# sanje2v/DualSuperResLearningForSemSeg

Measured on AMD Instinct MI355X. Metric: stage-3 train images/sec at 256x512->512x1024, higher is better.
Workload: dtype f32; 1 GPU; DSRL stage 3 (ResNet-101 OS16 + ASPP + SSSR/SISR decoders + FA loss), full train step, random-init weights, 256x512 input -> 512x1024 logits; global_batch=8, per_gpu_batch=8, parallelism=dp1, optimizer=SGD m0.9 wd5e-4 lr0.006

## Files before the change

### dualsuperreslearningforsemseg_amd/csrc/bn.hip

```cpp
#include "common.h"
#include <algorithm>
#include <initializer_list>
#include <atomic>
#include <mutex>
#include <stdlib.h>

struct SeedArg { unsigned long long value; const unsigned long long* dev; };

namespace dsrl {

constexpr int kMaxRowBlocks = 256;

static int row_blocks(int64_t P) { return (int)std::max<int64_t>(1, std::min<int64_t>(kMaxRowBlocks, ceil_div(P, 32))); }

__global__ __launch_bounds__(256) void bn_partial_kernel(const float* __restrict__ x, int ld, long long P, int C, long long rows_per_block,
                                                          float* __restrict__ part, int nbx) {
    __shared__ float sh[3][256];
    const ChanMap m = chan_map(C, blockIdx.y);
    const long long row0 = blockIdx.x * rows_per_block, row1 = min(P, row0 + rows_per_block);
    float n = 0.f, s1 = 0.f, s2 = 0.f, k0 = 0.f;
    if (m.c >= 0) {
        long long p = row0 + m.slot;
        if (p < row1) k0 = x[p * ld + m.c];
#pragma unroll 4
// ... 1465 lines not shown
                                  float* dresidual, int lddr, int64_t P, int C, const float* mean, const float* invstd, const float* gamma,
                                  float* dgamma, float* dbeta, int relu, float drop_p, int training, float* stats, int stats_parts, uint32_t* dx_amax,
                                  dsrl_stream_t stream, const BnRes2* res2);
extern "C" int dsrl_bn_bwd_from_stats_drop(const float* x, int ldx, const float* y, int ldy, const float* dy, int lddy, float* dx, int lddx,
                                           float* dresidual, int lddr, int64_t P, int C, const float* mean, const float* invstd, const float* gamma,
                                           float* dgamma, float* dbeta, int relu, float drop_p, int training, float* stats, int stats_parts, uint32_t* dx_amax,
                                           dsrl_stream_t stream) {
    return bn_bwd_from_stats_impl(x, ldx, y, ldy, dy, lddy, dx, lddx, dresidual, lddr, P, C, mean, invstd, gamma, dgamma, dbeta, relu, drop_p, training, stats, stats_parts,
                                  dx_amax, stream, nullptr);
}
extern "C" int dsrl_bn_bwd_from_stats_res(const float* x, int ldx, const float* y, int ldy, const float* dy, int lddy, float* dx, int lddx,
                                          float* dresidual, int lddr, int64_t P, int C, const float* mean, const float* invstd, const float* gamma,
                                          float* dgamma, float* dbeta, int relu, float drop_p, int training, float* stats, int stats_parts, uint32_t* dx_amax,
                                          const float* res_x, int res_ldx, const float* res_mean, const float* res_invstd, float* res_stats, int res_parts,
                                          dsrl_stream_t stream) {
    DSRL_REQUIRE(dresidual && res_x && res_mean && res_invstd && res_stats && res_ldx >= C && res_ldx % 4 == 0 && ((uintptr_t)res_x % 16) == 0, DSRL_E_BADARG,
                 "bn_bwd_from_stats_res: the residual branch's input / statistics / partials buffer are required (stride a multiple of 4, 16-byte aligned)");
    DSRL_REQUIRE(res_parts > 0 && res_parts == dsrl_bn_bwd_from_stats_res_parts(P, C, stats_parts), DSRL_E_BADARG,
                 "bn_bwd_from_stats_res: this launch writes %d row blocks of sums, the caller expects %d (dsrl_bn_bwd_from_stats_res_parts)",
                 dsrl_bn_bwd_from_stats_res_parts(P, C, stats_parts), res_parts);
    const BnRes2 r2{res_x, res_ldx, res_mean, res_invstd, res_stats, res_parts};
    return bn_bwd_from_stats_impl(x, ldx, y, ldy, dy, lddy, dx, lddx, dresidual, lddr, P, C, mean, invstd, gamma, dgamma, dbeta, relu, drop_p, training, stats, stats_parts,
                                  dx_amax, stream, &r2);
}
static int bn_bwd_from_stats_impl(const float* x, int ldx, const float* y, int ldy, const float* dy, int lddy, float* dx, int lddx,
                                  float* dresidual, int lddr, int64_t P, int C, const float* mean, const float* invstd, const float* gamma,
                                  float* dgamma, float* dbeta, int relu, float drop_p, int training, float* stats, int stats_parts, uint32_t* dx_amax,
                                  dsrl_stream_t stream, const BnRes2* res2) {
    DSRL_REQUIRE(drop_p >= 0.f && drop_p < 1.f && (drop_p == 0.f || relu), DSRL_E_BADARG, "bn_bwd_from_stats_drop: dropout p=%f needs the ReLU mask (y > 0)", drop_p);
    const float ks = drop_p > 0.f ? 1.f / (1.f - drop_p) : 1.f;
    DSRL_REQUIRE(x && dy && dx && mean && invstd && gamma && stats && P > 0 && P < (1ll << 31) && C > 0, DSRL_E_BADARG, "bn_bwd_from_stats: bad arguments");
// ... 100 lines not shown
```

### dualsuperreslearningforsemseg_amd/csrc/conv_common.h

```cpp
#pragma once
#include "common.h"

namespace dsrl {

using f32x16 = __attribute__((ext_vector_type(16))) float;
using bf16x8 = __attribute__((ext_vector_type(8))) __bf16;
using bf16x4 = __attribute__((ext_vector_type(4))) __bf16;
using f16x8 = __attribute__((ext_vector_type(8))) _Float16;
using f16x4 = __attribute__((ext_vector_type(4))) _Float16;

template <bool F16> struct Plane;
template <> struct Plane<false> {
    using v4 = bf16x4; using v8 = bf16x8;
    static __device__ __forceinline__ v4 cvt(const float* r) { return v4{(__bf16)r[0], (__bf16)r[1], (__bf16)r[2], (__bf16)r[3]}; }
    static __device__ __forceinline__ void residual(float* r, v4 t) {
#pragma unroll
        for (int e = 0; e < 4; ++e) r[e] -= (float)t[e];
    }
    static __device__ __forceinline__ f32x16 mfma(v8 a, v8 b, f32x16 c) { return __builtin_amdgcn_mfma_f32_32x32x16_bf16(a, b, c, 0, 0, 0); }
};
__device__ __forceinline__ float f16_resid_lo(unsigned t, float r) { float d; asm("v_fma_mix_f32 %0, %1, -1.0, %2 op_sel:[0,0,0] op_sel_hi:[1,0,0]" : "=v"(d) : "v"(t), "v"(r)); return d; }
__device__ __forceinline__ float f16_resid_hi(unsigned t, float r) { float d; asm("v_fma_mix_f32 %0, %1, -1.0, %2 op_sel:[1,0,0] op_sel_hi:[1,0,0]" : "=v"(d) : "v"(t), "v"(r)); return d; }
template <> struct Plane<true> {
    using v4 = f16x4; using v8 = f16x8;
// ... 27 lines not shown
    int R, S, Ho, Wo;
    int stride, pad, dil;
    int M;
    int cchunks;
    int splits;
    long long slab;
    unsigned x_bytes, w_bytes, y_bytes;
    int mtiles, ntiles, xcd_remap;
    int kg;
    int accumulate;
    float* stats;
    const float* bn_x; const float* bn_y; const float* bn_mean; const float* bn_invstd; float* bstats;
    int bn_ldx, bn_ldy, bn_relu;
    float bn_gscale;
    int bn_fast;
    int par, Hh, Wh, pbm;
    const unsigned* amax_a; const unsigned* amax_b;
    int w_split;
    unsigned mHW, sHW, mW, sW, mNT, sNT;
    unsigned a_lo, b_lo;
    int planes;
    float* coop_slab; unsigned* tickets;
};
constexpr int kCoopMaxTiles = (kAmaxShardStride - 1) * kAmaxShards;
__host__ __device__ inline int coop_ticket_word(int t) { return kAmaxShardStride * (t / (kAmaxShardStride - 1)) + 1 + t % (kAmaxShardStride - 1); }
__device__ __forceinline__ int dgrad_pix(const ConvArgs& a, int m) {
    const int t = m / a.pbm, p2 = a.par * a.par, c = t % p2, j = (t / p2) * a.pbm + (m - t * a.pbm);
    const int hw = a.Hh * a.Wh, n = j / hw, r = j - n * hw, hh = r / a.Wh, wh = r - hh * a.Wh;
    const int ph = c / a.par, pw = c - ph * a.par;
    return (n * a.Ho + hh * a.par + ph) * a.Wo + wh * a.par + pw;
// ... 54 lines not shown
```

### dualsuperreslearningforsemseg_amd/csrc/conv_igemm.hip

```cpp
#include "common.h"
#include "conv_common.h"
#include <algorithm>
#include <atomic>
#include <stdlib.h>
#include <string.h>
#include <mutex>
#include <vector>

namespace dsrl {

static std::atomic<int> g_conv_precision{-1};
constexpr int BK = 32;
constexpr int LDS_LD = 36;

template <int MR, int NR, int WGM, int WGN, bool DGRAD, int MINW = 2, bool = false>
__global__ __launch_bounds__(256, MINW) void conv_igemm_f32_kernel(const ConvArgs a) {
    constexpr int BM = 32 * MR * WGM, BN = 32 * NR * WGN;
    constexpr int A_IT = BM / 32, B_IT = BN / 32;
    extern __shared__ __attribute__((aligned(16))) float smem[];

    const int tid = threadIdx.x;
    const int lane = tid & 63;
    const int wave = __builtin_amdgcn_readfirstlane(tid >> 6);
    const int wm = wave / WGN, wn = wave % WGN;
// ... 1453 lines not shown
    if (int e = bind_stream_device(st)) return e;
    hipLaunchKernelGGL(weight_transpose_batched_kernel, dim3((unsigned)ceil_div(total_tiles, (int64_t)kWtTilesPerBlock)), dim3(256), 0, st, (const long long*)table, n,
                       (long long)total_tiles);
    return launch_status("weight_transpose_batched_kernel");
}

extern "C" int dsrl_conv2d_filters_amax_segment_floats(void) { return kAmaxSegFloats; }
extern "C" int dsrl_conv2d_filters_amax_batched(const int64_t* table, int64_t nseg, dsrl_stream_t stream) {
    DSRL_REQUIRE(table && nseg > 0 && nseg < (1ll << 31), DSRL_E_BADARG, "conv2d_filters_amax_batched: bad arguments");
    hipStream_t st = (hipStream_t)stream;
    if (int e = bind_stream_device(st)) return e;
    hipLaunchKernelGGL(weight_amax_batched_kernel, dim3((unsigned)nseg), dim3(256), 0, st, (const long long*)table);
    return launch_status("weight_amax_batched_kernel");
}

struct DgradBn { const float* x; const float* y; const float* mean; const float* invstd; float* stats; int ldx, ldy, relu; float gscale = 1.f; };
static bool bn_y_ok(const float* y, int ldy, int relu, int N, int H, int W, int C) {
    if (relu == 2) return y != nullptr && C % 32 == 0 && (long long)ldy >= (long long)N * H * W && ((uintptr_t)y % 4) == 0;
    return relu == 0 || (relu == 1 && y != nullptr && ldy >= C);
}
static int dgrad_impl(const float* dy, int lddy, const float* w, const float* wt_in, float* dx, int lddx,
                      int N, int H, int W, int C, int K, int R, int S, int stride, int pad, int dil,
                      void* ws, size_t ws_bytes, dsrl_stream_t stream, int accumulate, const DgradBn* bn = nullptr,
                      const unsigned* dy_amax = nullptr, const unsigned* w_amax = nullptr, const void* wt_split = nullptr,
                      const void* dy_planes = nullptr, const void* wt_planes = nullptr) {
    if (int e = check_conv(dy, w, dx, N, H, W, C, K, R, S, stride, pad, dil)) return e;
    const int Kp = pad4(K);
    DSRL_REQUIRE(lddy % 4 == 0 && ((uintptr_t)dy % 16) == 0, DSRL_E_UNSUPPORTED,
                 "conv2d_dgrad: lddy (%d) must be a multiple of 4 and dy 16-byte aligned", lddy);
    DSRL_REQUIRE(lddy >= Kp && lddx >= C, DSRL_E_BADARG, "conv2d_dgrad: ld smaller than (padded) channel count");
    hipStream_t st = (hipStream_t)stream;
// ... 50 lines not shown
                           (const float*)slabs, p.splits, a.slab, p.M, C, (const float*)nullptr, dx, lddx, accumulate);
        return launch_status("splitk_reduce_kernel");
    }
    if (p.splits > 1) {
        a.coop_slab = slabs; a.tickets = const_cast<unsigned*>(a.amax_a);
        a.y_bytes = (unsigned)span_bytes(p.M, lddx, C);
    }
    a.y = dx; a.ldy = lddx; a.bias = nullptr; a.accumulate = accumulate;
    if (stride > 1 && conv_planes(PASS_DGRAD) && H % stride == 0 && W % stride == 0 && (W / stride) % 32 == 0 && knob("DSRL_DGRAD_PARITY", 1)) {
        int bm, bn_; cfg_dims(p.cfg, bm, bn_);
        const long long Mc = (long long)N * (H / stride) * (W / stride);
        if (Mc % bm == 0) { a.par = stride; a.Hh = H / stride; a.Wh = W / stride; a.pbm = bm; }
    }
    if (bn) {
        a.bn_x = bn->x; a.bn_y = bn->y; a.bn_mean = bn->mean; a.bn_invstd = bn->invstd; a.bstats = bn->stats; a.bn_ldx = bn->ldx; a.bn_ldy = bn->ldy; a.bn_relu = bn->relu;
        a.bn_gscale = bn->gscale;
        const bool y4 = bn->relu != 1 || (bn->ldy % 4 == 0 && ((uintptr_t)bn->y % 16) == 0);
        a.bn_fast = a.par == 0 && C % 4 == 0 && bn->ldx % 4 == 0 && y4 && ((uintptr_t)bn->x % 16) == 0 &&
                    ((uintptr_t)bn->mean % 16) == 0 && ((uintptr_t)bn->invstd % 16) == 0 && ((uintptr_t)bn->stats % 16) == 0;
    }
    return launch_igemm<true>(a, p.cfg, st);
}

extern "C" int dsrl_conv2d_dgrad(const float* dy, int lddy, const float* w, const float* wt_in, float* dx, int lddx,
                                 int N, int H, int W, int C, int K, int R, int S, int stride, int pad, int dil,
                                 void* ws, size_t ws_bytes, dsrl_stream_t stream) {
    return dgrad_impl(dy, lddy, w, wt_in, dx, lddx, N, H, W, C, K, R, S, stride, pad, dil, ws, ws_bytes, stream, 0);
}
extern "C" int dsrl_conv2d_dgrad_stats_parts(int N, int H, int W, int C, int K, int R, int S, int stride, int pad, int dil) {
    const int Ho = out_size(H, R, stride, pad, dil), Wo = out_size(W, S, stride, pad, dil);
    if (Ho <= 0 || Wo <= 0) return 0;
    const int npl = conv_planes(PASS_DGRAD);
    return fwd_stats_parts(plan_dgrad(N, Ho, Wo, pad4(K), C, R, S, H, W, npl, stride), npl, true);
}
// ... 204 lines not shown
                 dsrl_conv2d_dgrad_stats_parts(N, H, W, C, K, R, S, stride, pad, dil), stats_parts);
    DgradBn bn{bn_x, bn_y, bn_mean, bn_invstd, bstats, bn_ldx, bn_ldy, bn_relu};
    return dgrad_impl(dy, lddy, w, wt_in, dx, lddx, N, H, W, C, K, R, S, stride, pad, dil, ws, ws_bytes, stream, accumulate ? 1 : 0, &bn, dy_amax, w_amax, wt_split);
}
extern "C" int dsrl_conv2d_fwd_planes(const float* x, int ldx, const uint32_t* x_amax, const void* x_planes, const float* w, const uint32_t* w_amax, const void* w_split,
                                      const void* w_planes, const float* bias, float* y, int ldy, int N, int H, int W, int C, int K, int R, int S, int stride, int pad, int dil,
                                      void* ws, size_t ws_bytes, float* stats, int stats_parts, dsrl_stream_t stream) {
    return fwd_impl(x, ldx, w, bias, y, ldy, N, H, W, C, K, R, S, stride, pad, dil, ws, ws_bytes, stream, stats, stats_parts, x_amax, w_amax, w_split, x_planes, w_planes);
}
extern "C" int dsrl_conv2d_dgrad_planes(const float* dy, int lddy, const uint32_t* dy_amax, const void* dy_planes, const float* w, const float* wt_in, const uint32_t* w_amax,
                                        const void* wt_split, const void* wt_planes, float* dx, int lddx,
                                        int N, int H, int W, int C, int K, int R, int S, int stride, int pad, int dil,
                                        void* ws, size_t ws_bytes, const float* bn_x, int bn_ldx, const float* bn_y, int bn_ldy,
                                        const float* bn_mean, const float* bn_invstd, int bn_relu, float* bstats, int stats_parts, int accumulate,
                                        dsrl_stream_t stream) {
    return dsrl_conv2d_dgrad_planes_drop(dy, lddy, dy_amax, dy_planes, w, wt_in, w_amax, wt_split, wt_planes, dx, lddx, N, H, W, C, K, R, S, stride, pad, dil, ws, ws_bytes,
                                         bn_x, bn_ldx, bn_y, bn_ldy, bn_mean, bn_invstd, bn_relu, 0.f, bstats, stats_parts, accumulate, stream);
}
extern "C" int dsrl_conv2d_dgrad_planes_drop(const float* dy, int lddy, const uint32_t* dy_amax, const void* dy_planes, const float* w, const float* wt_in, const uint32_t* w_amax,
                                             const void* wt_split, const void* wt_planes, float* dx, int lddx,
                                             int N, int H, int W, int C, int K, int R, int S, int stride, int pad, int dil,
                                             void* ws, size_t ws_bytes, const float* bn_x, int bn_ldx, const float* bn_y, int bn_ldy,
                                             const float* bn_mean, const float* bn_invstd, int bn_relu, float bn_drop_p, float* bstats, int stats_parts, int accumulate,
                                             dsrl_stream_t stream) {
    DSRL_REQUIRE(bn_drop_p >= 0.f && bn_drop_p < 1.f && (bn_drop_p == 0.f || bn_relu), DSRL_E_BADARG, "conv2d_dgrad_planes_drop: dropout p=%f needs the ReLU mask (y > 0)", bn_drop_p);
    if (bstats == nullptr)
        return dgrad_impl(dy, lddy, w, wt_in, dx, lddx, N, H, W, C, K, R, S, stride, pad, dil, ws, ws_bytes, stream, accumulate ? 1 : 0, nullptr, dy_amax, w_amax, wt_split,
                          dy_planes, wt_planes);
    DSRL_REQUIRE(bn_x && bn_mean && bn_invstd && bn_ldx >= C && bn_y_ok(bn_y, bn_ldy, bn_relu, N, H, W, C), DSRL_E_BADARG, "conv2d_dgrad_planes: bad BatchNorm arguments");
    DSRL_REQUIRE(dsrl_conv2d_dgrad_stats_parts(N, H, W, C, K, R, S, stride, pad, dil) == stats_parts && stats_parts > 0, DSRL_E_BADARG,
                 "conv2d_dgrad_planes: this launch writes %d row blocks of partials, the caller expects %d",
                 dsrl_conv2d_dgrad_stats_parts(N, H, W, C, K, R, S, stride, pad, dil), stats_parts);
    DgradBn bn{bn_x, bn_y, bn_mean, bn_invstd, bstats, bn_ldx, bn_ldy, bn_relu};
    bn.gscale = bn_drop_p > 0.f ? 1.f / (1.f - bn_drop_p) : 1.f;
    return dgrad_impl(dy, lddy, w, wt_in, dx, lddx, N, H, W, C, K, R, S, stride, pad, dil, ws, ws_bytes, stream, accumulate ? 1 : 0, &bn, dy_amax, w_amax, wt_split,
                      dy_planes, wt_planes);
}
extern "C" int dsrl_conv2d_wgrad_amax(const float* x, int ldx, const uint32_t* x_amax, const float* dy, int lddy, const uint32_t* dy_amax, float* dw,
                                      int N, int H, int W, int C, int K, int R, int S, int stride, int pad, int dil,
                                      void* ws, size_t ws_bytes, dsrl_stream_t stream) {
    return wgrad_impl(x, ldx, dy, lddy, dw, N, H, W, C, K, R, S, stride, pad, dil, ws, ws_bytes, stream, x_amax, dy_amax);
}


namespace dsrl {
constexpr unsigned kGroupMagic = 0x44535247u;
constexpr int kGroupMaxProblems = 512, kGroupMaxLaunches = kNumCfg + 2;
constexpr int kCfgW3 = kNumCfg;
struct GroupLaunch { int cfg, first, count, grid; double flops, bytes; };
// ... 332 lines not shown
```

### dualsuperreslearningforsemseg_amd/csrc/conv_planes.hip

```cpp
#include "common.h"
#include "conv_common.h"
#include "lds_dma.h"
#include <algorithm>

namespace dsrl {

template <int NPL> struct PlaneMfma;
template <> struct PlaneMfma<2> {
    template <int MR, int NR>
    static __device__ __forceinline__ void run(f32x16 (&acc)[MR][NR], const f16x8 (&fa)[MR][2], const f16x8 (&fb)[NR][2]) {
#pragma unroll
        for (int sum = 1; sum >= 0; --sum)
#pragma unroll
            for (int pa = 0; pa <= sum; ++pa)
#pragma unroll
                for (int i = 0; i < MR; ++i)
#pragma unroll
                    for (int j = 0; j < NR; ++j)
                        acc[i][j] = __builtin_amdgcn_mfma_f32_32x32x16_f16(fa[i][pa], fb[j][sum - pa], acc[i][j], 0, 0, 0);
    }
};
template <> struct PlaneMfma<1> {
    template <int MR, int NR>
    static __device__ __forceinline__ void run(f32x16 (&acc)[MR][NR], const f16x8 (&fa)[MR][1], const f16x8 (&fb)[NR][1]) {
// ... 276 lines not shown
        const float bv = (a.bias != nullptr && kok) ? a.bias[k] : 0.f;
#pragma unroll
        for (int i = 0; i < MR; ++i) {
            const int mb32 = m0 + (wm * MR + i) * 32, mb = mb32 + rq;
            if (a.accumulate && a.splits == 1) {
                float old[EPG];
#pragma unroll
                for (int e = 0; e < EPG; ++e) {
                    const int m = mb + (e & 3) + 8 * (e >> 2);
                    const unsigned off = (kok && m < a.M) ? ((unsigned)m * (unsigned)a.ldy + (unsigned)k) * 4u : kOOB;
                    old[e] = __uint_as_float(__builtin_amdgcn_raw_buffer_load_b32(yr, (int)off, 0, 0));
                }
#pragma unroll
                for (int e = 0; e < EPG; ++e) share_add(i, j, e, old[e]);
            }
#pragma unroll
            for (int e = 0; e < EPG; ++e) {
                const int m = mb + (e & 3) + 8 * (e >> 2);
                const unsigned off = (kok && m < a.M) ? ((unsigned)m * (unsigned)a.ldy + (unsigned)k) * 4u : kOOB;
                __builtin_amdgcn_raw_buffer_store_b32(__float_as_uint(share(i, j, e) + bv), yr, (int)off, 0, 0);
            }
        }
    }
    bool bstats_done = false;
    if constexpr (DGRAD && KG == 1) {
        if (a.bstats != nullptr && (a.splits == 1) && a.bn_fast) {
            constexpr int TR = 32 * MR, TC = 32 * NR, CQ = TC / 4, RSTEP = 64 / CQ, NIT = TR / RSTEP, NB = NIT < 8 ? NIT : 8;
            float* wt = reinterpret_cast<float*>(smem) + (size_t)wave * TR * TC;
            __syncthreads();
#pragma unroll
// ... 21 lines not shown
                    if (a.bn_relu == 2) yv[u] = bn_mask4(ok ? bn_mask_word(a, kk, m) >> (kk & 31) : 15u);
                    else yv[u] = (ok && a.bn_relu) ? *reinterpret_cast<const float4*>(a.bn_y + (long long)m * a.bn_ldy + kk) : make_float4(1.f, 1.f, 1.f, 1.f);
                }
#pragma unroll
                for (int u = 0; u < NB; ++u) {
                    const int row = r0_ + RSTEP * (b0 + u);
                    if (kok4 && mrow0 + row < a.M) {
                        const float4 gv = *reinterpret_cast<const float4*>(wt + row * TC + 4 * c4);
                        const float gs = a.bn_gscale;
                        const float g0 = (a.bn_relu && !(yv[u].x > 0.f)) ? 0.f : gv.x * gs, g1 = (a.bn_relu && !(yv[u].y > 0.f)) ? 0.f : gv.y * gs;
                        const float g2 = (a.bn_relu && !(yv[u].z > 0.f)) ? 0.f : gv.z * gs, g3 = (a.bn_relu && !(yv[u].w > 0.f)) ? 0.f : gv.w * gs;
                        sg[0] += g0; sgx[0] += g0 * ((xv[u].x - mu4.x) * is4.x);
                        sg[1] += g1; sgx[1] += g1 * ((xv[u].y - mu4.y) * is4.y);
                        sg[2] += g2; sgx[2] += g2 * ((xv[u].z - mu4.z) * is4.z);
                        sg[3] += g3; sgx[3] += g3 * ((xv[u].w - mu4.w) * is4.w);
                    }
                }
            }
#pragma unroll
            for (int sft = CQ; sft < 64; sft <<= 1)
#pragma unroll
                for (int q = 0; q < 4; ++q) { sg[q] += __shfl_xor(sg[q], sft); sgx[q] += __shfl_xor(sgx[q], sft); }
            if (lane < CQ && kok4) {
                const int nparts = a.mtiles * WGM, part = tile_m * WGM + wm;
                float* o = a.bstats + (long long)part * a.K + kk;
                *reinterpret_cast<float4*>(o) = make_float4(sg[0], sg[1], sg[2], sg[3]);
                *reinterpret_cast<float4*>(o + (long long)nparts * a.K) = make_float4(sgx[0], sgx[1], sgx[2], sgx[3]);
            }
            bstats_done = true;
        }
// ... 14 lines not shown
#pragma unroll
                for (int e = 0; e < EPG; ++e) {
                    const int m = mb32 + rq + (e & 3) + 8 * (e >> 2);
                    const bool ok = kok && m < a.M;
                    const long long px = m;
                    xv[e] = ok ? a.bn_x[px * a.bn_ldx + k] : 0.f;
                    if (a.bn_relu == 2) yv[e] = (!ok || ((bn_mask_word(a, k, px) >> (k & 31)) & 1u)) ? 1.f : 0.f;
                    else yv[e] = (ok && a.bn_relu) ? a.bn_y[px * a.bn_ldy + k] : 1.f;
                }
#pragma unroll
                for (int e = 0; e < EPG; ++e) {
                    const int m = mb32 + rq + (e & 3) + 8 * (e >> 2);
                    if (kok && m < a.M) {
                        const float g = (a.bn_relu && !(yv[e] > 0.f)) ? 0.f : share(i, j, e) * a.bn_gscale;
                        sg += g; sgx += g * ((xv[e] - mu) * is);
                    }
                }
            }
            sg += __shfl_xor(sg, 32); sgx += __shfl_xor(sgx, 32);
            if (KG == 1) {
                if (lane < 32 && kok) {
                    float* o = a.bstats + (long long)part * a.K + k;
                    o[0] = sg; o[(long long)nparts * a.K] = sgx;
                }
            } else if (lane < 32) {
                ex[(((grp * NW + wave) * NR + j) * 2 + 0) * 32 + lane] = sg;
                ex[(((grp * NW + wave) * NR + j) * 2 + 1) * 32 + lane] = sgx;
            }
        }
        if constexpr (KG > 1) {
// ... 282 lines not shown
```

### dualsuperreslearningforsemseg_amd/csrc/conv_split_kernel.h

```cpp
#pragma once
#include "common.h"
#include "conv_common.h"

namespace dsrl {

template <int MR, int NR, int WGM, int WGN, bool DGRAD, int NPL, int KG = 1, int ARITH = 0, bool STR1 = false, bool COOP = false>
__global__ __launch_bounds__(64 * WGM * WGN * KG, KG == 1 ? 2 : 1)
void conv_igemm_split_kernel(const ConvArgs a) {
    const int stride = STR1 ? 1 : a.stride, par = STR1 ? 0 : a.par;
    constexpr bool F16 = ARITH != 0, PREB = ARITH == 2;
    constexpr int NT = 64 * WGM * WGN, RP = NT / 4;
    static_assert(NT == 256 || (NT == 512 && KG == 1), "4 waves per K group, or one group of 8 waves");
    static_assert(!F16 || NPL <= 2, "f16x3 carries two fp16 terms per operand, f16x1 one");
    using PT = Plane<F16>;
    using pl4 = typename PT::v4; using pl8 = typename PT::v8;
    const unsigned am_a = F16 ? amax_fetch(a.amax_a) : 0u, am_b = F16 ? amax_fetch(a.amax_b) : 0u;
    int sh_a = 0, sh_b = 0;
    constexpr int BM = 32 * MR * WGM, BN = 32 * NR * WGN;
    constexpr int A_IT = (BM + RP - 1) / RP, B_IT = (BN + RP - 1) / RP;
    constexpr int NV = A_IT + B_IT;
    constexpr bool FS = F16;
    constexpr int ROWB = FS ? 64 : 32;
    constexpr int STAGE = (BM + BN) * NPL * ROWB;
    extern __shared__ __attribute__((aligned(16))) float smem[];
// ... 444 lines not shown
#pragma unroll
        for (int i = 0; i < MR; ++i) {
            const int mb32 = m0 + (wm * MR + i) * 32, mb = mb32 + rq;
            const int pix0 = (DGRAD && par) ? dgrad_pix(a, min(mb32, a.M - 1)) : mb32, pst = (DGRAD && par) ? par : 1;
            if (a.accumulate && single) {
                float old[EPG];
#pragma unroll
                for (int e = 0; e < EPG; ++e) {
                    const int m = mb + (e & 3) + 8 * (e >> 2);
                    const unsigned off = (kok && m < a.M) ? ((unsigned)(pix0 + (m - mb32) * pst) * (unsigned)a.ldy + (unsigned)k) * 4u : kOOB;
                    old[e] = __uint_as_float(__builtin_amdgcn_raw_buffer_load_b32(yr, (int)off, 0, 0));
                }
#pragma unroll
                for (int e = 0; e < EPG; ++e) share_add(i, j, e, old[e]);
            }
#pragma unroll
            for (int e = 0; e < EPG; ++e) {
                const int m = mb + (e & 3) + 8 * (e >> 2);
                const unsigned off = (kok && m < a.M) ? ((unsigned)(pix0 + (m - mb32) * pst) * (unsigned)a.ldy + (unsigned)k) * 4u : kOOB;
                __builtin_amdgcn_raw_buffer_store_b32(__float_as_uint(share(i, j, e) + bv), yr, (int)off, 0, 0);
            }
        }
    }
    bool bstats_done = false;
    if constexpr (DGRAD && KG == 1) {
        if (a.bstats != nullptr && single && a.bn_fast) {
            constexpr int TR = 32 * MR, TC = 32 * NR, CQ = TC / 4, RSTEP = 64 / CQ, NIT = TR / RSTEP, NB = NIT < 8 ? NIT : 8;
            float* wt = reinterpret_cast<float*>(smem) + (size_t)wave * TR * TC;
            __syncthreads();
#pragma unroll
// ... 21 lines not shown
                    if (a.bn_relu == 2) yv[u] = bn_mask4(ok ? bn_mask_word(a, kk, m) >> (kk & 31) : 15u);
                    else yv[u] = (ok && a.bn_relu) ? *reinterpret_cast<const float4*>(a.bn_y + (long long)m * a.bn_ldy + kk) : make_float4(1.f, 1.f, 1.f, 1.f);
                }
#pragma unroll
                for (int u = 0; u < NB; ++u) {
                    const int row = r0_ + RSTEP * (b0 + u);
                    if (kok4 && mrow0 + row < a.M) {
                        const float4 gv = *reinterpret_cast<const float4*>(wt + row * TC + 4 * c4);
                        const float gs = a.bn_gscale;
                        const float g0 = (a.bn_relu && !(yv[u].x > 0.f)) ? 0.f : gv.x * gs, g1 = (a.bn_relu && !(yv[u].y > 0.f)) ? 0.f : gv.y * gs;
                        const float g2 = (a.bn_relu && !(yv[u].z > 0.f)) ? 0.f : gv.z * gs, g3 = (a.bn_relu && !(yv[u].w > 0.f)) ? 0.f : gv.w * gs;
                        sg[0] += g0; sgx[0] += g0 * ((xv[u].x - mu4.x) * is4.x);
                        sg[1] += g1; sgx[1] += g1 * ((xv[u].y - mu4.y) * is4.y);
                        sg[2] += g2; sgx[2] += g2 * ((xv[u].z - mu4.z) * is4.z);
                        sg[3] += g3; sgx[3] += g3 * ((xv[u].w - mu4.w) * is4.w);
                    }
                }
            }
#pragma unroll
            for (int sft = CQ; sft < 64; sft <<= 1)
#pragma unroll
                for (int q = 0; q < 4; ++q) { sg[q] += __shfl_xor(sg[q], sft); sgx[q] += __shfl_xor(sgx[q], sft); }
            if (lane < CQ && kok4) {
                const int nparts = a.mtiles * WGM, part = tile_m * WGM + wm;
                float* o = a.bstats + (long long)part * a.K + kk;
                *reinterpret_cast<float4*>(o) = make_float4(sg[0], sg[1], sg[2], sg[3]);
                *reinterpret_cast<float4*>(o + (long long)nparts * a.K) = make_float4(sgx[0], sgx[1], sgx[2], sgx[3]);
            }
            bstats_done = true;
        }
// ... 15 lines not shown
#pragma unroll
                for (int e = 0; e < EPG; ++e) {
                    const int m = mb32 + rq + (e & 3) + 8 * (e >> 2);
                    const bool ok = kok && m < a.M;
                    const long long px = pix0 + (m - mb32) * pst;
                    xv[e] = ok ? a.bn_x[px * a.bn_ldx + k] : 0.f;
                    if (a.bn_relu == 2) yv[e] = (!ok || ((bn_mask_word(a, k, px) >> (k & 31)) & 1u)) ? 1.f : 0.f;
                    else yv[e] = (ok && a.bn_relu) ? a.bn_y[px * a.bn_ldy + k] : 1.f;
                }
#pragma unroll
                for (int e = 0; e < EPG; ++e) {
                    const int m = mb32 + rq + (e & 3) + 8 * (e >> 2);
                    if (kok && m < a.M) {
                        const float g = (a.bn_relu && !(yv[e] > 0.f)) ? 0.f : share(i, j, e) * a.bn_gscale;
                        sg += g; sgx += g * ((xv[e] - mu) * is);
                    }
                }
            }
            sg += __shfl_xor(sg, 32); sgx += __shfl_xor(sgx, 32);
            if (KG == 1) {
                if (lane < 32 && kok) {
                    float* o = a.bstats + (long long)part * a.K + k;
                    o[0] = sg; o[(long long)nparts * a.K] = sgx;
                }
            } else if (lane < 32) {
                ex[(((grp * 4 + wave) * NR + j) * 2 + 0) * 32 + lane] = sg;
                ex[(((grp * 4 + wave) * NR + j) * 2 + 1) * 32 + lane] = sgx;
            }
        }
        if constexpr (KG > 1) {
// ... 80 lines not shown
```

### dualsuperreslearningforsemseg_amd/functional.py

```python
import contextlib
import ctypes
import math
import os
import sys
import weakref

import numpy as np

import torch

from . import _lib
from ._lib import call, knob, query, DsrlHipError

CL = torch.channels_last


_raw_stream = getattr(torch._C, '_cuda_getCurrentRawStream', None)
_raw_device = getattr(torch._C, '_cuda_getDevice', None)


def _stream():
    if _raw_stream is not None and _raw_device is not None:
        return _raw_stream(_raw_device())
    return torch.cuda.current_stream().cuda_stream
# ... 549 lines not shown
grad_slots_enabled = knob('DSRL_GRAD_SLOTS', True)
outer_grad_slot = knob('DSRL_OUTER_SLOT', True)


class GradSlot:
    __slots__ = ('buf', 'closed', 'link')

    def __init__(self):
        self.buf, self.closed = None, False
        self.link = None


bn_bwd_stats_enabled = knob('DSRL_BN_BWD_STATS', True)
bn_bwd_stats_shared = knob('DSRL_BN_BWD_STATS_SHARED', True)
bn_mask_enabled = knob('DSRL_BN_MASK', True)


class BNLink:
    __slots__ = ('x', 'y_ptr', 'y_shape', 'mean', 'invstd', 'relu', 'valid', 'stats', 'parts', 'dx_ptr', 'shared', 'drop_p', 'mask')

    def __init__(self, shared=False):
        self.x = self.mean = self.invstd = self.stats = None
        self.y_ptr, self.y_shape = 0, None
        self.relu, self.valid, self.parts, self.dx_ptr = False, False, 0, 0
        self.shared = shared
        self.drop_p = 0.0
        self.mask = None


class _Fork(torch.autograd.Function):
    @staticmethod
    def forward(ctx, x):
        return x.view_as(x)

    @staticmethod
    def backward(ctx, g):
        return g


def fork(x):
    y = _Fork.apply(x)
    a = carried_amax(x)
# ... 89 lines not shown
                ctx.wparam._dsrl_arena.written(ctx.wparam, side)
            else:
                dw = sink if sink is not None else torch.empty((K, Cc, R, S), device=x.device, dtype=torch.float32, memory_format=CL)
                ws = _ws(cquery('dsrl_conv2d_wgrad_workspace_bytes', *shp), x)
                call('dsrl_conv2d_wgrad_amax', x.data_ptr(), ldx, p_(xa), dy.data_ptr(), lddy, p_(dya), dw.data_ptr(), *shp, ws.data_ptr(), ws.numel(), st)
                if sink is not None:
                    ctx.wparam._dsrl_arena.written(ctx.wparam)
                    dw = None
        if ctx.needs_input_grad[0]:
            slot = ctx.gslot
            acc = (slot is not None and not slot.closed and slot.buf is not None and tuple(slot.buf.shape) == (N, Cc, H, W)
                   and slot.buf.is_contiguous(memory_format=CL))
            dx = slot.buf if acc else new_cl((N, Cc, H, W), x)
            if slot is not None and slot.link is not None and slot.link is not ctx.in_link and slot.link.stats is not None:
                slot.link.stats = None
            ws = _ws(cquery('dsrl_conv2d_dgrad_workspace_bytes', *shp), x)
            wt_ptr = None
            if ctx.wparam is not None:
                h = getattr(ctx.wparam, '_dsrl_operands', None)
                wt = None if h is None else h[0].fp32_transpose(h[1])
                if wt is not None:
                    wt_ptr = wt.data_ptr()
            link = ctx.in_link
            parts = 0
            final = (not acc and ctx.gslot is None) or (acc and getattr(link, 'shared', False))
            if (link is not None and link.valid and final and link.y_ptr == x.data_ptr() and link.y_shape == (N, Cc, H, W) and Cc % 32 == 0):
                parts = int(query('dsrl_conv2d_dgrad_stats_parts', *shp))
            if parts > 0:
                bstats = torch.empty(cquery('dsrl_bn_stats_floats', 2, parts, Cc), device=x.device, dtype=torch.float32)
                _, bld = pm(link.x)
                ym = (link.mask.data_ptr(), N * H * W, 2) if (link.mask is not None and link.relu) else (x.data_ptr(), ldx, int(link.relu))
                call('dsrl_conv2d_dgrad_planes_drop', dy.data_ptr(), lddy, p_(dya), p_(dyp), w.data_ptr(), wt_ptr, p_(wa), p_(wtsp), p_(wtpl), dx.data_ptr(), Cc, *shp,
                     ws.data_ptr(), ws.numel(), link.x.data_ptr(), bld, ym[0], ym[1], link.mean.data_ptr(), link.invstd.data_ptr(), ym[2],
                     float(link.drop_p), bstats.data_ptr(), parts, int(acc), st)
                link.stats, link.parts, link.dx_ptr = bstats, parts, dx.data_ptr()
            else:
                call('dsrl_conv2d_dgrad_planes', dy.data_ptr(), lddy, p_(dya), p_(dyp), w.data_ptr(), wt_ptr, p_(wa), p_(wtsp), p_(wtpl), dx.data_ptr(), Cc, *shp,
                     ws.data_ptr(), ws.numel(), None, 0, None, 0, None, None, 0, None, 0, int(acc), st)
            if acc:
                dx = None
            elif slot is not None:
                if slot.buf is None:
                    slot.buf = dx
                else:
                    slot.closed = True
        if ctx.has_bias and ctx.needs_input_grad[2]:
            P = dy.shape[0] * dy.shape[2] * dy.shape[3]
            bsink = _sink_flat(ctx.bparam, K)
            db = bsink if bsink is not None else torch.empty(K, device=x.device, dtype=torch.float32)
            ws = _ws(cquery('dsrl_colsum_workspace_bytes', P, K), x)
# ... 112 lines not shown
        else:
            mean = running_mean
            invstd = frozen_invstd(running_var, eps)
            if invstd is None:
                invstd = torch.empty(Cc, device=x.device, dtype=torch.float32)
                call('dsrl_bn_invstd_from_var', running_var.data_ptr(), Cc, float(eps), invstd.data_ptr(), st)
            call('dsrl_bn_apply', x.data_ptr(), ldx, y.data_ptr(), Cc, P, Cc, mean.data_ptr(), invstd.data_ptr(), gamma.data_ptr(), beta.data_ptr(),
                 res_ptr, ldr, int(relu), float(drop_p), int(seed), int(rng_stream), ya_ptr, st)
        if ya is not None:
            set_amax(y, ya)
        ctx.save_for_backward(x, y, mean, invstd, gamma)
        ctx.mask = mask
        if out_link is not None and (drop_p == 0.0 or relu) and Cc % 32 == 0 and ldx == Cc:
            out_link.x, out_link.mean, out_link.invstd, out_link.relu, out_link.valid = x, mean, invstd, bool(relu), True
            out_link.mask = mask
            out_link.y_ptr, out_link.y_shape, out_link.drop_p = y.data_ptr(), tuple(y.shape), float(drop_p)
        ctx.cfg = (bool(training), bool(relu), float(drop_p), residual is not None)
        ctx.gb = (gamma, beta) if isinstance(gamma, torch.nn.Parameter) and isinstance(beta, torch.nn.Parameter) else None
        return y

    @staticmethod
    def backward(ctx, dy):
        x, y, mean, invstd, gamma = ctx.saved_tensors
        training, relu, drop_p, has_res = ctx.cfg
        dy, lddy = pm(dy)
        _, ldx = pm(x)
        N, Cc, H, W = x.shape
        P = N * H * W
        dx = new_cl((N, Cc, H, W), x)
        dres = new_cl((N, Cc, H, W), x) if has_res else None
        sg = sb = None
        if ctx.gb is not None and ctx.needs_input_grad[1] and ctx.needs_input_grad[2]:
            sg = _sink(ctx.gb[0])
            sb = _sink(ctx.gb[1]) if sg is not None else None
        dgamma = sg if sg is not None else torch.empty(Cc, device=x.device, dtype=torch.float32)
        dbeta = sb if sb is not None else torch.empty(Cc, device=x.device, dtype=torch.float32)
        dxa = amax_slot(x.device) if f16_mode() else None
        dxa_ptr = None if dxa is None else dxa.data_ptr()
        link = ctx.out_link
        if link is not None and link.stats is not None and link.dx_ptr == dy.data_ptr() and lddy == Cc and (drop_p == 0.0 or relu):
            rl = ctx.res_link
            ym = (ctx.mask.data_ptr(), P, 2) if (ctx.mask is not None and relu) else (y.data_ptr(), Cc, int(relu))
            rparts = int(query('dsrl_bn_bwd_from_stats_res_parts', P, Cc, int(link.parts))) if (rl is not None and dres is not None and bn_res_stats_enabled) else 0
            if rparts > 0:
                rstats = torch.empty(cquery('dsrl_bn_stats_floats', 2, rparts, Cc), device=x.device, dtype=torch.float32)
                _, rld = pm(rl.x)
                call('dsrl_bn_bwd_from_stats_res', x.data_ptr(), ldx, ym[0], ym[1], dy.data_ptr(), lddy, dx.data_ptr(), Cc, dres.data_ptr(), Cc, P, Cc,
                     mean.data_ptr(), invstd.data_ptr(), gamma.data_ptr(), dgamma.data_ptr(), dbeta.data_ptr(), ym[2], float(drop_p), int(training),
                     link.stats.data_ptr(), int(link.parts), dxa_ptr, rl.x.data_ptr(), rld, rl.mean.data_ptr(), rl.invstd.data_ptr(), rstats.data_ptr(), rparts, _stream())
                rl.stats, rl.parts, rl.dx_ptr = rstats, rparts, dres.data_ptr()
            else:
                call('dsrl_bn_bwd_from_stats_drop', x.data_ptr(), ldx, ym[0], ym[1], dy.data_ptr(), lddy, dx.data_ptr(), Cc,
                     None if dres is None else dres.data_ptr(), Cc, P, Cc, mean.data_ptr(), invstd.data_ptr(), gamma.data_ptr(),
                     dgamma.data_ptr(), dbeta.data_ptr(), ym[2], float(drop_p), int(training), link.stats.data_ptr(), int(link.parts), dxa_ptr, _stream())
        else:
            ws = _ws(cquery('dsrl_bn_workspace_bytes', P, Cc), x)
            call('dsrl_bn_bwd', x.data_ptr(), ldx, y.data_ptr(), Cc, dy.data_ptr(), lddy, dx.data_ptr(), Cc,
                 None if dres is None else dres.data_ptr(), Cc, P, Cc, mean.data_ptr(), invstd.data_ptr(), gamma.data_ptr(),
                 dgamma.data_ptr(), dbeta.data_ptr(), int(relu), drop_p, int(training), ws.data_ptr(), ws.numel(), dxa_ptr, _stream())
        if dxa is not None:
            set_amax(dx, dxa)
        if sg is not None:
            ctx.gb[0]._dsrl_arena.written(ctx.gb[0]); dgamma = None
        if sb is not None:
            ctx.gb[1]._dsrl_arena.written(ctx.gb[1]); dbeta = None
        if dres is not None and ctx.rslot is not None:
            if ctx.rslot.buf is None:
                ctx.rslot.buf = dres
# ... 1376 lines not shown
```

### include/dsrl_hip.h

```cpp
#ifndef DSRL_HIP_H
#define DSRL_HIP_H

#include <stddef.h>
#include <stdint.h>

#ifdef __cplusplus
extern "C" {
#endif

#define DSRL_ABI_VERSION 1

#define DSRL_OK 0
#define DSRL_E_BADARG (-1)
#define DSRL_E_UNSUPPORTED (-2)
#define DSRL_E_WORKSPACE (-3)
#define DSRL_E_LAUNCH (-4)

typedef void* dsrl_stream_t;

int dsrl_version(void);
const char* dsrl_last_error(void);
int dsrl_device_check(int* cu_count);

size_t dsrl_conv2d_fwd_workspace_bytes(int N, int H, int W, int C, int K, int R, int S, int stride, int pad, int dil);
// ... 50 lines not shown
                           dsrl_stream_t stream);
size_t dsrl_planes_lo_offset(int64_t elems);
size_t dsrl_planes_bytes(int64_t elems, int nplanes);
int dsrl_split_planes(const float* x, int ld, int64_t P, int C, const uint32_t* amax, void* planes, int nplanes, dsrl_stream_t stream);
int dsrl_conv2d_filter_planes_batched(const int64_t* table, int n, int64_t total_tiles, dsrl_stream_t stream);
int dsrl_conv2d_fwd_planes(const float* x, int ldx, const uint32_t* x_amax, const void* x_planes , const float* w, const uint32_t* w_amax,
                           const void* w_split , const void* w_planes , const float* bias , float* y, int ldy,
                           int N, int H, int W, int C, int K, int R, int S, int stride, int pad, int dil,
                           void* ws, size_t ws_bytes, float* stats , int stats_parts, dsrl_stream_t stream);
int dsrl_conv2d_dgrad_planes(const float* dy, int lddy, const uint32_t* dy_amax, const void* dy_planes , const float* w, const float* wt ,
                             const uint32_t* w_amax, const void* wt_split , const void* wt_planes , float* dx, int lddx,
                             int N, int H, int W, int C, int K, int R, int S, int stride, int pad, int dil,
                             void* ws, size_t ws_bytes, const float* bn_x, int bn_ldx, const float* bn_y, int bn_ldy,
                             const float* bn_mean, const float* bn_invstd, int bn_relu, float* bstats , int stats_parts, int accumulate,
                             dsrl_stream_t stream);
int dsrl_conv2d_dgrad_planes_drop(const float* dy, int lddy, const uint32_t* dy_amax, const void* dy_planes , const float* w, const float* wt ,
                             const uint32_t* w_amax, const void* wt_split , const void* wt_planes , float* dx, int lddx,
                             int N, int H, int W, int C, int K, int R, int S, int stride, int pad, int dil,
                             void* ws, size_t ws_bytes, const float* bn_x, int bn_ldx, const float* bn_y, int bn_ldy,
                             const float* bn_mean, const float* bn_invstd, int bn_relu, float bn_drop_p, float* bstats , int stats_parts, int accumulate,
                             dsrl_stream_t stream);
int dsrl_conv2d_wgrad_amax(const float* x, int ldx, const uint32_t* x_amax, const float* dy, int lddy, const uint32_t* dy_amax, float* dw,
                           int N, int H, int W, int C, int K, int R, int S, int stride, int pad, int dil,
                           void* ws, size_t ws_bytes, dsrl_stream_t stream);
int dsrl_conv_precision(int mode);
int64_t dsrl_conv2d_inbounds_macs(int N, int H, int W, int C, int K, int R, int S, int stride, int pad, int dil);

size_t dsrl_conv2d_rowfold_fwd_workspace_bytes(int N, int H, int W, int Cfold, int K, int R, int stride, int Ho, int Wo);
int dsrl_conv2d_rowfold_fwd(const float* x, int ldx, const float* w, const float* bias , float* y, int ldy,
                            int N, int H, int W, int Cfold, int K, int R, int stride, int Ho, int Wo, int64_t algorithmic_macs,
// ... 36 lines not shown
int dsrl_bn_bwd(const float* x, int ldx, const float* y, int ldy, const float* dy, int lddy,
                float* dx, int lddx, float* dresidual , int lddr, int64_t P, int C,
                const float* mean, const float* invstd, const float* gamma,
                float* dgamma, float* dbeta, int relu, float drop_p, int training,
                void* ws, size_t ws_bytes, uint32_t* dx_amax , dsrl_stream_t stream);
int dsrl_bn_bwd_from_stats(const float* x, int ldx, const float* y , int ldy, const float* dy, int lddy, float* dx, int lddx,
                           float* dresidual , int lddr, int64_t P, int C, const float* mean, const float* invstd, const float* gamma,
                           float* dgamma , float* dbeta , int relu, int training, float* stats, int stats_parts,
                           uint32_t* dx_amax , dsrl_stream_t stream);
int dsrl_bn_bwd_from_stats_drop(const float* x, int ldx, const float* y , int ldy, const float* dy, int lddy, float* dx, int lddx,
                           float* dresidual , int lddr, int64_t P, int C, const float* mean, const float* invstd, const float* gamma,
                           float* dgamma , float* dbeta , int relu, float drop_p, int training, float* stats, int stats_parts,
                           uint32_t* dx_amax , dsrl_stream_t stream);
int dsrl_bn_bwd_from_stats_res_parts(int64_t P, int C, int stats_parts);
int dsrl_bn_bwd_from_stats_res(const float* x, int ldx, const float* y , int ldy, const float* dy, int lddy, float* dx, int lddx,
                           float* dresidual, int lddr, int64_t P, int C, const float* mean, const float* invstd, const float* gamma,
                           float* dgamma , float* dbeta , int relu, float drop_p, int training, float* stats, int stats_parts,
                           uint32_t* dx_amax , const float* res_x, int res_ldx, const float* res_mean, const float* res_invstd,
                           float* res_stats, int res_parts, dsrl_stream_t stream);

int dsrl_rng_bind_device_key(const uint64_t* dev_key );
int dsrl_rng_advance_key(uint64_t* state , dsrl_stream_t stream);

int dsrl_dropout_fwd(const float* x, int ldx, float* y, int ldy, int64_t P, int C, float p, uint64_t seed, uint32_t rng_stream, dsrl_stream_t stream);
int dsrl_dropout_bwd(const float* dy, int lddy, float* dx, int lddx, int64_t P, int C, float p, uint64_t seed, uint32_t rng_stream, dsrl_stream_t stream);

int dsrl_bilinear_ac_fwd(const float* x, int ldx, float* y, int ldy, int N, int H, int W, int C, int Ho, int Wo, dsrl_stream_t stream);
size_t dsrl_bilinear_ac_bwd_workspace_bytes(int N, int H, int W, int C, int Ho, int Wo);
int dsrl_bilinear_ac_bwd(const float* dy, int lddy, float* dx, int lddx, int N, int H, int W, int C, int Ho, int Wo,
                         void* ws, size_t ws_bytes, dsrl_stream_t stream);
int dsrl_global_avgpool_fwd(const float* x, int ldx, float* y, int N, int HW, int C, dsrl_stream_t stream);
// ... 242 lines not shown
```

Measured before the change: 512.1 images/s.

## Write ReLU-masked residual gradient in-place from dgrad epilogue

When a BatchNorm+ReLU output feeds a residual add, the dgrad epilogue that already computes the BN sums now also stores the ReLU-masked gradient back into the dy buffer. The BN backward then reuses that buffer as the residual gradient instead of allocating and writing a separate dres tensor. This removes one full-size allocation and write per residual block. In exchange the epilogue does extra stores, and the store skips the normal dx write path when the flag is set.

New measurement: 515.8 images/s (median of 6 runs). No clear change (+0.7%).

```diff
diff --git a/dualsuperreslearningforsemseg_amd/csrc/bn.hip b/dualsuperreslearningforsemseg_amd/csrc/bn.hip
--- a/dualsuperreslearningforsemseg_amd/csrc/bn.hip
+++ b/dualsuperreslearningforsemseg_amd/csrc/bn.hip
@@ -1503,7 +1503,7 @@
                                           float* dgamma, float* dbeta, int relu, float drop_p, int training, float* stats, int stats_parts, uint32_t* dx_amax,
                                           const float* res_x, int res_ldx, const float* res_mean, const float* res_invstd, float* res_stats, int res_parts,
                                           dsrl_stream_t stream) {
-    DSRL_REQUIRE(dresidual && res_x && res_mean && res_invstd && res_stats && res_ldx >= C && res_ldx % 4 == 0 && ((uintptr_t)res_x % 16) == 0, DSRL_E_BADARG,
+    DSRL_REQUIRE(res_x && res_mean && res_invstd && res_stats && res_ldx >= C && res_ldx % 4 == 0 && ((uintptr_t)res_x % 16) == 0, DSRL_E_BADARG,
                  "bn_bwd_from_stats_res: the residual branch's input / statistics / partials buffer are required (stride a multiple of 4, 16-byte aligned)");
     DSRL_REQUIRE(res_parts > 0 && res_parts == dsrl_bn_bwd_from_stats_res_parts(P, C, stats_parts), DSRL_E_BADARG,
                  "bn_bwd_from_stats_res: this launch writes %d row blocks of sums, the caller expects %d (dsrl_bn_bwd_from_stats_res_parts)",
diff --git a/dualsuperreslearningforsemseg_amd/csrc/conv_common.h b/dualsuperreslearningforsemseg_amd/csrc/conv_common.h
--- a/dualsuperreslearningforsemseg_amd/csrc/conv_common.h
+++ b/dualsuperreslearningforsemseg_amd/csrc/conv_common.h
@@ -65,6 +65,7 @@
     int bn_ldx, bn_ldy, bn_relu;
     float bn_gscale;
     int bn_fast;
+    int bn_store;
     int par, Hh, Wh, pbm;
     const unsigned* amax_a; const unsigned* amax_b;
     int w_split;
diff --git a/dualsuperreslearningforsemseg_amd/csrc/conv_igemm.hip b/dualsuperreslearningforsemseg_amd/csrc/conv_igemm.hip
--- a/dualsuperreslearningforsemseg_amd/csrc/conv_igemm.hip
+++ b/dualsuperreslearningforsemseg_amd/csrc/conv_igemm.hip
@@ -1491,7 +1491,7 @@
     return launch_status("weight_amax_batched_kernel");
 }
 
-struct DgradBn { const float* x; const float* y; const float* mean; const float* invstd; float* stats; int ldx, ldy, relu; float gscale = 1.f; };
+struct DgradBn { const float* x; const float* y; const float* mean; const float* invstd; float* stats; int ldx, ldy, relu; float gscale = 1.f; int store = 0; };
 static bool bn_y_ok(const float* y, int ldy, int relu, int N, int H, int W, int C) {
     if (relu == 2) return y != nullptr && C % 32 == 0 && (long long)ldy >= (long long)N * H * W && ((uintptr_t)y % 4) == 0;
     return relu == 0 || (relu == 1 && y != nullptr && ldy >= C);
@@ -1572,10 +1572,11 @@
     }
     if (bn) {
         a.bn_x = bn->x; a.bn_y = bn->y; a.bn_mean = bn->mean; a.bn_invstd = bn->invstd; a.bstats = bn->stats; a.bn_ldx = bn->ldx; a.bn_ldy = bn->ldy; a.bn_relu = bn->relu;
-        a.bn_gscale = bn->gscale;
+        a.bn_gscale = bn->gscale; a.bn_store = bn->store;
         const bool y4 = bn->relu != 1 || (bn->ldy % 4 == 0 && ((uintptr_t)bn->y % 16) == 0);
         a.bn_fast = a.par == 0 && C % 4 == 0 && bn->ldx % 4 == 0 && y4 && ((uintptr_t)bn->x % 16) == 0 &&
-                    ((uintptr_t)bn->mean % 16) == 0 && ((uintptr_t)bn->invstd % 16) == 0 && ((uintptr_t)bn->stats % 16) == 0;
+                    ((uintptr_t)bn->mean % 16) == 0 && ((uintptr_t)bn->invstd % 16) == 0 && ((uintptr_t)bn->stats % 16) == 0 &&
+                    (!bn->store || (lddx % 4 == 0 && ((uintptr_t)dx % 16) == 0));
     }
     return launch_igemm<true>(a, p.cfg, st);
 }
@@ -1810,6 +1811,7 @@
                                         void* ws, size_t ws_bytes, const float* bn_x, int bn_ldx, const float* bn_y, int bn_ldy,
                                         const float* bn_mean, const float* bn_invstd, int bn_relu, float* bstats, int stats_parts, int accumulate,
                                         dsrl_stream_t stream) {
+    DSRL_REQUIRE(bstats == nullptr || (bn_relu >= 0 && bn_relu <= 2), DSRL_E_BADARG, "conv2d_dgrad_planes: relu = %d (0, 1, or 2 = y is the sign mask)", bn_relu);
     return dsrl_conv2d_dgrad_planes_drop(dy, lddy, dy_amax, dy_planes, w, wt_in, w_amax, wt_split, wt_planes, dx, lddx, N, H, W, C, K, R, S, stride, pad, dil, ws, ws_bytes,
                                          bn_x, bn_ldx, bn_y, bn_ldy, bn_mean, bn_invstd, bn_relu, 0.f, bstats, stats_parts, accumulate, stream);
 }
@@ -1820,6 +1822,12 @@
                                              const float* bn_mean, const float* bn_invstd, int bn_relu, float bn_drop_p, float* bstats, int stats_parts, int accumulate,
                                              dsrl_stream_t stream) {
     DSRL_REQUIRE(bn_drop_p >= 0.f && bn_drop_p < 1.f && (bn_drop_p == 0.f || bn_relu), DSRL_E_BADARG, "conv2d_dgrad_planes_drop: dropout p=%f needs the ReLU mask (y > 0)", bn_drop_p);
+    const int store_masked = (bn_relu & DSRL_BN_STORE_MASKED) != 0 && bn_relu > 0;
+    if (store_masked) {
+        bn_relu &= ~DSRL_BN_STORE_MASKED;
+        DSRL_REQUIRE(bstats != nullptr && (bn_relu == 1 || bn_relu == 2) && bn_drop_p == 0.f, DSRL_E_BADARG,
+                     "conv2d_dgrad_planes_drop: the masked store needs the BatchNorm sums (bstats), a ReLU mask (relu 1 or 2) and no dropout (relu = %d, p = %f)", bn_relu, bn_drop_p);
+    }
     if (bstats == nullptr)
         return dgrad_impl(dy, lddy, w, wt_in, dx, lddx, N, H, W, C, K, R, S, stride, pad, dil, ws, ws_bytes, stream, accumulate ? 1 : 0, nullptr, dy_amax, w_amax, wt_split,
                           dy_planes, wt_planes);
@@ -1829,6 +1837,7 @@
                  dsrl_conv2d_dgrad_stats_parts(N, H, W, C, K, R, S, stride, pad, dil), stats_parts);
     DgradBn bn{bn_x, bn_y, bn_mean, bn_invstd, bstats, bn_ldx, bn_ldy, bn_relu};
     bn.gscale = bn_drop_p > 0.f ? 1.f / (1.f - bn_drop_p) : 1.f;
+    bn.store = store_masked;
     return dgrad_impl(dy, lddy, w, wt_in, dx, lddx, N, H, W, C, K, R, S, stride, pad, dil, ws, ws_bytes, stream, accumulate ? 1 : 0, &bn, dy_amax, w_amax, wt_split,
                       dy_planes, wt_planes);
 }
diff --git a/dualsuperreslearningforsemseg_amd/csrc/conv_planes.hip b/dualsuperreslearningforsemseg_amd/csrc/conv_planes.hip
--- a/dualsuperreslearningforsemseg_amd/csrc/conv_planes.hip
+++ b/dualsuperreslearningforsemseg_amd/csrc/conv_planes.hip
@@ -314,6 +314,7 @@
 #pragma unroll
                 for (int e = 0; e < EPG; ++e) share_add(i, j, e, old[e]);
             }
+            if (DGRAD && a.bn_store) continue;
 #pragma unroll
             for (int e = 0; e < EPG; ++e) {
                 const int m = mb + (e & 3) + 8 * (e >> 2);
@@ -365,6 +366,11 @@
                         sg[1] += g1; sgx[1] += g1 * ((xv[u].y - mu4.y) * is4.y);
                         sg[2] += g2; sgx[2] += g2 * ((xv[u].z - mu4.z) * is4.z);
                         sg[3] += g3; sgx[3] += g3 * ((xv[u].w - mu4.w) * is4.w);
+                        if (a.bn_store) {
+                            const u32x4 q = {__float_as_uint(yv[u].x > 0.f ? gv.x + 0.f : 0.f), __float_as_uint(yv[u].y > 0.f ? gv.y + 0.f : 0.f),
+                                             __float_as_uint(yv[u].z > 0.f ? gv.z + 0.f : 0.f), __float_as_uint(yv[u].w > 0.f ? gv.w + 0.f : 0.f)};
+                            __builtin_amdgcn_raw_buffer_store_b128(q, yr, (int)(((unsigned)(mrow0 + row) * (unsigned)a.ldy + (unsigned)kk) * 4u), 0, 0);
+                        }
                     }
                 }
             }
@@ -409,6 +415,9 @@
                     if (kok && m < a.M) {
                         const float g = (a.bn_relu && !(yv[e] > 0.f)) ? 0.f : share(i, j, e) * a.bn_gscale;
                         sg += g; sgx += g * ((xv[e] - mu) * is);
+                        if (a.bn_store)
+                            __builtin_amdgcn_raw_buffer_store_b32(__float_as_uint(yv[e] > 0.f ? share(i, j, e) + 0.f : 0.f), yr,
+                                                                  (int)(((unsigned)m * (unsigned)a.ldy + (unsigned)k) * 4u), 0, 0);
                     }
                 }
             }
diff --git a/dualsuperreslearningforsemseg_amd/csrc/conv_split_kernel.h b/dualsuperreslearningforsemseg_amd/csrc/conv_split_kernel.h
--- a/dualsuperreslearningforsemseg_amd/csrc/conv_split_kernel.h
+++ b/dualsuperreslearningforsemseg_amd/csrc/conv_split_kernel.h
@@ -482,6 +482,7 @@
 #pragma unroll
                 for (int e = 0; e < EPG; ++e) share_add(i, j, e, old[e]);
             }
+            if (DGRAD && a.bn_store) continue;
 #pragma unroll
             for (int e = 0; e < EPG; ++e) {
                 const int m = mb + (e & 3) + 8 * (e >> 2);
@@ -533,6 +534,11 @@
                         sg[1] += g1; sgx[1] += g1 * ((xv[u].y - mu4.y) * is4.y);
                         sg[2] += g2; sgx[2] += g2 * ((xv[u].z - mu4.z) * is4.z);
                         sg[3] += g3; sgx[3] += g3 * ((xv[u].w - mu4.w) * is4.w);
+                        if (a.bn_store) {
+                            const u32x4 q = {__float_as_uint(yv[u].x > 0.f ? gv.x + 0.f : 0.f), __float_as_uint(yv[u].y > 0.f ? gv.y + 0.f : 0.f),
+                                             __float_as_uint(yv[u].z > 0.f ? gv.z + 0.f : 0.f), __float_as_uint(yv[u].w > 0.f ? gv.w + 0.f : 0.f)};
+                            __builtin_amdgcn_raw_buffer_store_b128(q, yr, (int)(((unsigned)(mrow0 + row) * (unsigned)a.ldy + (unsigned)kk) * 4u), 0, 0);
+                        }
                     }
                 }
             }
@@ -578,6 +584,9 @@
                     if (kok && m < a.M) {
                         const float g = (a.bn_relu && !(yv[e] > 0.f)) ? 0.f : share(i, j, e) * a.bn_gscale;
                         sg += g; sgx += g * ((xv[e] - mu) * is);
+                        if (a.bn_store)
+                            __builtin_amdgcn_raw_buffer_store_b32(__float_as_uint(yv[e] > 0.f ? share(i, j, e) + 0.f : 0.f), yr,
+                                                                  (int)(((unsigned)(pix0 + (m - mb32) * pst) * (unsigned)a.ldy + (unsigned)k) * 4u), 0, 0);
                     }
                 }
             }
diff --git a/dualsuperreslearningforsemseg_amd/functional.py b/dualsuperreslearningforsemseg_amd/functional.py
--- a/dualsuperreslearningforsemseg_amd/functional.py
+++ b/dualsuperreslearningforsemseg_amd/functional.py
@@ -587,10 +587,12 @@
 bn_bwd_stats_enabled = knob('DSRL_BN_BWD_STATS', True)
 bn_bwd_stats_shared = knob('DSRL_BN_BWD_STATS_SHARED', True)
 bn_mask_enabled = knob('DSRL_BN_MASK', True)
+res_inplace_enabled = knob('DSRL_RES_INPLACE', True)
+DSRL_BN_STORE_MASKED = 4
 
 
 class BNLink:
-    __slots__ = ('x', 'y_ptr', 'y_shape', 'mean', 'invstd', 'relu', 'valid', 'stats', 'parts', 'dx_ptr', 'shared', 'drop_p', 'mask')
+    __slots__ = ('x', 'y_ptr', 'y_shape', 'mean', 'invstd', 'relu', 'valid', 'stats', 'parts', 'dx_ptr', 'shared', 'drop_p', 'mask', 'wants_masked', 'masked')
 
     def __init__(self, shared=False):
         self.x = self.mean = self.invstd = self.stats = None
@@ -599,6 +601,8 @@
         self.shared = shared
         self.drop_p = 0.0
         self.mask = None
+        self.wants_masked = False
+        self.masked = False
 
 
 class _Fork(torch.autograd.Function):
@@ -718,6 +722,7 @@
             dx = slot.buf if acc else new_cl((N, Cc, H, W), x)
             if slot is not None and slot.link is not None and slot.link is not ctx.in_link and slot.link.stats is not None:
                 slot.link.stats = None
+                slot.link.masked = False
             ws = _ws(cquery('dsrl_conv2d_dgrad_workspace_bytes', *shp), x)
             wt_ptr = None
             if ctx.wparam is not None:
@@ -734,10 +739,11 @@
                 bstats = torch.empty(cquery('dsrl_bn_stats_floats', 2, parts, Cc), device=x.device, dtype=torch.float32)
                 _, bld = pm(link.x)
                 ym = (link.mask.data_ptr(), N * H * W, 2) if (link.mask is not None and link.relu) else (x.data_ptr(), ldx, int(link.relu))
+                masked = bool(link.wants_masked and link.relu and link.drop_p == 0.0 and res_inplace_enabled)
                 call('dsrl_conv2d_dgrad_planes_drop', dy.data_ptr(), lddy, p_(dya), p_(dyp), w.data_ptr(), wt_ptr, p_(wa), p_(wtsp), p_(wtpl), dx.data_ptr(), Cc, *shp,
-                     ws.data_ptr(), ws.numel(), link.x.data_ptr(), bld, ym[0], ym[1], link.mean.data_ptr(), link.invstd.data_ptr(), ym[2],
-                     float(link.drop_p), bstats.data_ptr(), parts, int(acc), st)
-                link.stats, link.parts, link.dx_ptr = bstats, parts, dx.data_ptr()
+                     ws.data_ptr(), ws.numel(), link.x.data_ptr(), bld, ym[0], ym[1], link.mean.data_ptr(), link.invstd.data_ptr(),
+                     ym[2] | (DSRL_BN_STORE_MASKED if masked else 0), float(link.drop_p), bstats.data_ptr(), parts, int(acc), st)
+                link.stats, link.parts, link.dx_ptr, link.masked = bstats, parts, dx.data_ptr(), masked
             else:
                 call('dsrl_conv2d_dgrad_planes', dy.data_ptr(), lddy, p_(dya), p_(dyp), w.data_ptr(), wt_ptr, p_(wa), p_(wtsp), p_(wtpl), dx.data_ptr(), Cc, *shp,
                      ws.data_ptr(), ws.numel(), None, 0, None, 0, None, None, 0, None, 0, int(acc), st)
@@ -880,6 +886,8 @@
         if out_link is not None and (drop_p == 0.0 or relu) and Cc % 32 == 0 and ldx == Cc:
             out_link.x, out_link.mean, out_link.invstd, out_link.relu, out_link.valid = x, mean, invstd, bool(relu), True
             out_link.mask = mask
+            out_link.wants_masked = bool(training and relu and residual is not None and drop_p == 0.0 and res_inplace_enabled)
+            out_link.masked = False
             out_link.y_ptr, out_link.y_shape, out_link.drop_p = y.data_ptr(), tuple(y.shape), float(drop_p)
         ctx.cfg = (bool(training), bool(relu), float(drop_p), residual is not None)
         ctx.gb = (gamma, beta) if isinstance(gamma, torch.nn.Parameter) and isinstance(beta, torch.nn.Parameter) else None
@@ -894,7 +902,11 @@
         N, Cc, H, W = x.shape
         P = N * H * W
         dx = new_cl((N, Cc, H, W), x)
-        dres = new_cl((N, Cc, H, W), x) if has_res else None
+        link = ctx.out_link
+        linked = link is not None and link.stats is not None and link.dx_ptr == dy.data_ptr() and lddy == Cc and (drop_p == 0.0 or relu)
+        inplace = bool(linked and link.masked and has_res and relu and drop_p == 0.0 and res_inplace_enabled)
+        dres = (dy if inplace else new_cl((N, Cc, H, W), x)) if has_res else None
+        dres_ptr = None if (dres is None or inplace) else dres.data_ptr()
         sg = sb = None
         if ctx.gb is not None and ctx.needs_input_grad[1] and ctx.needs_input_grad[2]:
             sg = _sink(ctx.gb[0])
@@ -903,21 +915,20 @@
         dbeta = sb if sb is not None else torch.empty(Cc, device=x.device, dtype=torch.float32)
         dxa = amax_slot(x.device) if f16_mode() else None
         dxa_ptr = None if dxa is None else dxa.data_ptr()
-        link = ctx.out_link
-        if link is not None and link.stats is not None and link.dx_ptr == dy.data_ptr() and lddy == Cc and (drop_p == 0.0 or relu):
+        if linked:
             rl = ctx.res_link
             ym = (ctx.mask.data_ptr(), P, 2) if (ctx.mask is not None and relu) else (y.data_ptr(), Cc, int(relu))
             rparts = int(query('dsrl_bn_bwd_from_stats_res_parts', P, Cc, int(link.parts))) if (rl is not None and dres is not None and bn_res_stats_enabled) else 0
             if rparts > 0:
                 rstats = torch.empty(cquery('dsrl_bn_stats_floats', 2, rparts, Cc), device=x.device, dtype=torch.float32)
                 _, rld = pm(rl.x)
-                call('dsrl_bn_bwd_from_stats_res', x.data_ptr(), ldx, ym[0], ym[1], dy.data_ptr(), lddy, dx.data_ptr(), Cc, dres.data_ptr(), Cc, P, Cc,
+                call('dsrl_bn_bwd_from_stats_res', x.data_ptr(), ldx, ym[0], ym[1], dy.data_ptr(), lddy, dx.data_ptr(), Cc, dres_ptr, Cc, P, Cc,
                      mean.data_ptr(), invstd.data_ptr(), gamma.data_ptr(), dgamma.data_ptr(), dbeta.data_ptr(), ym[2], float(drop_p), int(training),
                      link.stats.data_ptr(), int(link.parts), dxa_ptr, rl.x.data_ptr(), rld, rl.mean.data_ptr(), rl.invstd.data_ptr(), rstats.data_ptr(), rparts, _stream())
                 rl.stats, rl.parts, rl.dx_ptr = rstats, rparts, dres.data_ptr()
             else:
                 call('dsrl_bn_bwd_from_stats_drop', x.data_ptr(), ldx, ym[0], ym[1], dy.data_ptr(), lddy, dx.data_ptr(), Cc,
-                     None if dres is None else dres.data_ptr(), Cc, P, Cc, mean.data_ptr(), invstd.data_ptr(), gamma.data_ptr(),
+                     dres_ptr, Cc, P, Cc, mean.data_ptr(), invstd.data_ptr(), gamma.data_ptr(),
                      dgamma.data_ptr(), dbeta.data_ptr(), ym[2], float(drop_p), int(training), link.stats.data_ptr(), int(link.parts), dxa_ptr, _stream())
         else:
             ws = _ws(cquery('dsrl_bn_workspace_bytes', P, Cc), x)
diff --git a/include/dsrl_hip.h b/include/dsrl_hip.h
--- a/include/dsrl_hip.h
+++ b/include/dsrl_hip.h
@@ -88,6 +88,7 @@
                              void* ws, size_t ws_bytes, const float* bn_x, int bn_ldx, const float* bn_y, int bn_ldy,
                              const float* bn_mean, const float* bn_invstd, int bn_relu, float* bstats , int stats_parts, int accumulate,
                              dsrl_stream_t stream);
+#define DSRL_BN_STORE_MASKED 4
 int dsrl_conv2d_dgrad_planes_drop(const float* dy, int lddy, const uint32_t* dy_amax, const void* dy_planes , const float* w, const float* wt ,
                              const uint32_t* w_amax, const void* wt_split , const void* wt_planes , float* dx, int lddx,
                              int N, int H, int W, int C, int K, int R, int S, int stride, int pad, int dil,
@@ -154,7 +155,7 @@
                            uint32_t* dx_amax , dsrl_stream_t stream);
 int dsrl_bn_bwd_from_stats_res_parts(int64_t P, int C, int stats_parts);
 int dsrl_bn_bwd_from_stats_res(const float* x, int ldx, const float* y , int ldy, const float* dy, int lddy, float* dx, int lddx,
-                           float* dresidual, int lddr, int64_t P, int C, const float* mean, const float* invstd, const float* gamma,
+                           float* dresidual , int lddr, int64_t P, int C, const float* mean, const float* invstd, const float* gamma,
                            float* dgamma , float* dbeta , int relu, float drop_p, int training, float* stats, int stats_parts,
                            uint32_t* dx_amax , const float* res_x, int res_ldx, const float* res_mean, const float* res_invstd,
                            float* res_stats, int res_parts, dsrl_stream_t stream);
```
